# ColumbiaDVMM/ColumbiaImageSearch

Hardware: AMD Instinct MI355X
Metric: queries/sec @ recall@10 on 10M LOPQ index (higher is better)
Workload: dtype f64

## Files before the change

columbiaimagesearch_amd/csrc/lopq_scan3.hip:

```cpp
#include "scan_common.h"
#include <cmath>
#include <cstdio>
#include <cstdlib>

typedef unsigned short u16x2_t __attribute__((ext_vector_type(2)));

static __device__ __forceinline__ uint32_t pk_add_u16(uint32_t a, uint32_t b) {
    return __builtin_bit_cast(uint32_t, (u16x2_t)(__builtin_bit_cast(u16x2_t, a) + __builtin_bit_cast(u16x2_t, b)));
}
static __device__ __forceinline__ uint32_t pk_subsat_u16(uint32_t a, uint32_t b) {
    return __builtin_bit_cast(uint32_t, __builtin_elementwise_sub_sat(__builtin_bit_cast(u16x2_t, a), __builtin_bit_cast(u16x2_t, b)));
}

static __device__ __forceinline__ uint32_t pk_min_u16(uint32_t a, uint32_t b) {
    return __builtin_bit_cast(uint32_t, __builtin_elementwise_min(__builtin_bit_cast(u16x2_t, a), __builtin_bit_cast(u16x2_t, b)));
}

static const int S3G = 4;

#ifdef CIS_S3_COUNTERS
__device__ unsigned long long g_s3_ctr[16];
#define S3_CLK() ((long long)__builtin_amdgcn_s_memtime())
#define S3_CTR(i, v) do { if (threadIdx.x == 0) atomicAdd(&g_s3_ctr[i], (unsigned long long)(v)); } while (0)
extern "C" int cis_debug_counters3(unsigned long long* out, int reset) {
// ... 561 lines not shown
            for (int g = 0; g < G; ++g) {
                const uint32_t sg = (g & 1) ? (d[u][g >> 1] >> 16) : (d[u][g >> 1] & 0xffffu);
                const uint32_t t1 = (g & 1) ? ((g >> 1) ? s23 >> 16 : s01 >> 16) : ((g >> 1) ? s23 & 0xffffu : s01 & 0xffffu);
                pm[u][g] = __ballot(sg < t1) & anym[u];
                if (any_dup) {
                    bool same = true;
#pragma unroll
                    for (int i = 0; i < (M + 3) / 4; ++i) same = same && (cur[u].w[i] == dup[g].w[i]);
                    pm[u][g] &= ~(__ballot(same) & (has_dup[g] ? ~0ull : 0ull));
                }
            }
        }
#pragma unroll
        for (int g = 0; g < G; ++g) {
            if (g >= ng) break;
            uint32_t* rk = rk_all + (g * NW + w) * R;
            int ntot = 0;
#pragma unroll
            for (int u = 0; u < U; ++u) ntot += __popcll(pm[u][g]);
            if (ntot == 0) continue;
            auto entry = [&](int u) -> uint32_t {
                const uint32_t sg = (g & 1) ? (d[u][g >> 1] >> 16) : (d[u][g >> 1] & 0xffffu);
                return (sg << 16) | (uint32_t)(base + u * 64 + lane);
            };
            if (cnt[g] + ntot <= R) {
                int c = cnt[g];
#pragma unroll
                for (int u = 0; u < U; ++u) {
                    const unsigned long long m = pm[u][g];
                    if (m == 0ull) continue;
                    const int idx = __builtin_amdgcn_mbcnt_hi((unsigned)(m >> 32), __builtin_amdgcn_mbcnt_lo((unsigned)m, c));
                    if ((m >> lane) & 1ull) rk[idx] = entry(u);
                    c += __popcll(m);
                }
                cnt[g] = c;
                continue;
            }
            int u0 = 0;
            while (true) {
                bool full = false;
#pragma unroll
                for (int u = 0; u < U; ++u) {
                    const unsigned long long m = pm[u][g];
                    if (u < u0 || full || m == 0ull) continue;
                    const int n = __popcll(m);
                    if (cnt[g] + n > R) {
                        full = true;
                        u0 = u;
                        continue;
                    }
                    const int idx = cnt[g] + __builtin_amdgcn_mbcnt_hi((unsigned)(m >> 32), __builtin_amdgcn_mbcnt_lo((unsigned)m, 0));
                    if ((m >> lane) & 1ull) rk[idx] = entry(u);
                    cnt[g] += n;
                    u0 = u + 1;
                }
                if (!full) break;
                const QScale qsg = load_scale(&sh[g]);
                int c2 = wave_compact3<M, NR, NW>(rk, cnt[g], L, Lw, R - 64, qsg, &sh[g], w);
                if (c2 < 0) {
                    uint32_t dp = 0xffffffffu;
                    const WorkItem itg = items[item_idx[g]];
                    c2 = wave_compact3_exact<M, NR, NW>(rk, cnt[g], L, Lw, qsg, &sh[g], w, codes, start, K,
                                                        T + (int64_t)itg.tab0 * nf * K, T + (int64_t)itg.tab1 * nf * K, dp);
                    dp = (uint32_t)__builtin_amdgcn_readfirstlane((int)dp);
                    if (dp != 0xffffffffu) {
                        dup[g] = load_code<M>(codes, start + (int64_t)dp);
                        has_dup[g] = true;
                        any_dup = true;
                    }
                }
                cnt[g] = c2;
                const uint32_t thg = lds_ld(&sh[g].thr);
                if (lane == 0) st16(&thr1[g], thg + 1u);
                const unsigned long long dup_on = has_dup[g] ? ~0ull : 0ull;
#pragma unroll
                for (int u = 0; u < U; ++u) {
                    const uint32_t sg = (g & 1) ? (d[u][g >> 1] >> 16) : (d[u][g >> 1] & 0xffffu);
                    bool same = true;
#pragma unroll
                    for (int i = 0; i < (M + 3) / 4; ++i) same = same && (cur[u].w[i] == dup[g].w[i]);
                    pm[u][g] &= __ballot(sg <= thg) & ~(__ballot(same) & dup_on);
                }
            }
        }
    }
    S3_CTR(4, S3_CLK() - c0);
#pragma unroll
    for (int g = 0; g < G; ++g) {
        if (g >= ng) break;
        uint32_t* rk = rk_all + (g * NW + w) * R;
        if (cnt[g] > 0) cnt[g] = wave_compact3<M, NR, NW>(rk, cnt[g], L, Lw, NR * 64, load_scale(&sh[g]), &sh[g], w);
    }
    S3_CTR(5, S3_CLK() - c0);
    if constexpr (NW > 1) __syncthreads();
    S3_CTR(6, S3_CLK() - c0);
#pragma unroll
    for (int g = 0; g < G; ++g) {
        if (g >= ng) break;
        uint32_t* rk = rk_all + (g * NW + w) * R;
        const QScale qsg = load_scale(&sh[g]);
        if constexpr (NW > 1) cnt[g] = wave_filter3<NR, NW>(rk, cnt[g], qsg, &sh[g]);
        if (lane == 0) sh[g].wcnt[w] = cnt[g];
        if (tid == 0) {
            const uint64_t b = block_bound<NW>(&sh[g]);
            if (b < sh[g].ext) atomicMin(&qbound[items[item_idx[g]].q], (unsigned long long)b);
        }
    }
    if constexpr (NW > 1) __syncthreads();
#pragma unroll
    for (int g = 0; g < G; ++g) {
        if (g >= ng) break;
        const uint32_t* rk = rk_all + (g * NW + w) * R;
        int off = 0, total = 0;
#pragma unroll
        for (int i = 0; i < NW; ++i) {
            const int c = (NW > 1) ? sh[g].wcnt[i] : cnt[g];
            off += (i < w) ? c : 0;
            total += c;
        }
        uint64_t* out = item_surv + (int64_t)item_idx[g] * S + off;
        for (int e = lane; e < cnt[g]; e += 64) {
            const uint32_t x = rk[e];
            out[e] = ((uint64_t)(x >> 16) << 32) | (x & 0xffffu);
        }
        if (tid == 0) item_n[item_idx[g]] = total;
    }
    S3_CTR(7, S3_CLK() - c0);
    S3_CTR(0, 1);
}

template <int M, int NR, int U, int NW, int WPE>
__global__ __launch_bounds__(NW * 64) __attribute__((amdgpu_waves_per_eu(WPE, WPE))) void k_adc_scan3(
    const WorkItem* __restrict__ items, const TabDesc* __restrict__ tabs, const int* __restrict__ slots,
    const int* __restrict__ n_slots_ptr, const double* __restrict__ T, const float* __restrict__ T32,
    const uint8_t* __restrict__ codes, int K, int L, int S, int* __restrict__ queue_ctr ,
    uint64_t* __restrict__ item_surv, int* __restrict__ item_n, float* __restrict__ item_slack,
    unsigned long long* __restrict__ qbound , int two_pass, int single_queue ) {
    extern __shared__ __attribute__((aligned(16))) char smem[];
    constexpr int G = S3G;
    constexpr int R = NR * 64 - 8;
    int* s_next = reinterpret_cast<int*>(smem + (size_t)K * M * G * 2 + (size_t)G * NW * R * 4 + G * sizeof(Scan3Shared) + 32);
    const int* qs = n_slots_ptr + 8;
    const int home = blockIdx.x & 7;
    const long long k0 = S3_CLK();
    (void)k0;
    for (int a = 0; a < 8; ++a) {
        const int x = (home + a) & 7;
        const int qstart = qs[x];
        const int count = single_queue ? (x == 0 ? qs[1] - qstart : 0) : qs[x + 1] - qstart;
        if (count <= 0) continue;
        while (true) {
            const long long q0 = S3_CLK();
            (void)q0;
            int j;
            if constexpr (NW > 1) {
                __syncthreads();
                if (threadIdx.x == 0) *s_next = atomicAdd(&queue_ctr[x], 1);
                __syncthreads();
                j = __builtin_amdgcn_readfirstlane(*s_next);
            } else {
                int t = 0;
                if (threadIdx.x == 0) t = atomicAdd(&queue_ctr[x], 1);
                j = __builtin_amdgcn_readfirstlane(t);
            }
            S3_CTR(8, S3_CLK() - q0);
            if (j >= count) break;
            const int slot = qstart + j;
            int idx[G];
            int ng = 0;
            bool same = true;
#pragma unroll
            for (int g = 0; g < G; ++g) {
                idx[g] = slots[slot * G + g];
                if (idx[g] >= 0) {
                    ng = g + 1;
                    same = same && items[idx[g]].start == items[idx[0]].start && items[idx[g]].len == items[idx[0]].len;
                } else {
                    idx[g] = idx[0];
                }
            }
            if (!same) {
                for (int g2 = 0; g2 < ng; ++g2) {
                    int oi[G];
#pragma unroll
                    for (int g = 0; g < G; ++g) {
                        oi[g] = idx[0];
#pragma unroll
                        for (int gg = 1; gg < G; ++gg)
                            if (gg == g2) oi[g] = idx[gg];
                    }
                    if (g2 > 0) __syncthreads();
                    scan3_group<M, NR, U, NW>(items, tabs, oi, 1, T, T32, codes, K, L, S, item_surv, item_n, item_slack, qbound, smem, two_pass != 0);
                }
                continue;
            }
            scan3_group<M, NR, U, NW>(items, tabs, idx, ng, T, T32, codes, K, L, S, item_surv, item_n, item_slack, qbound, smem, two_pass != 0);
        }
    }
    S3_CTR(9, S3_CLK() - k0);
    S3_CTR(10, 1);
}

struct Slot4 {
    int item[S3G], tab0[S3G], tab1[S3G], q[S3G];
    float qinv[S3G];
    int start_lo, start_hi, len, ng;
    int ist_lo[S3G], ist_hi[S3G], ilen[S3G];
};
struct Scan4Shared {
    double inv_up, ub;
    uint64_t ext;
    uint32_t tau;
    int verify;
    int cnt;
    int q;
};

template <int M, int UU, int OCT = (M >= 8 ? 8 : 4)>
__device__ __forceinline__ void adc16_rows(const CodeWords<M> (&cur)[UU], const char* __restrict__ tab, const RotConsts<M>& rc,
                                           u32x2_t (&d)[UU]) {
    constexpr int NU = M / OCT;
    u32x2_t fbuf[2][OCT];
    uint32_t D[2][(M + 3) / 4];
    rot_words<M>(cur[0], rc, D[0]);
    adc16_issue<M, OCT>(D[0], 0, tab, rc, fbuf[0]);
#pragma unroll
    for (int q = 0; q < UU * NU; ++q) {
        const int u = q / NU, o = q % NU;
        if (q + 1 < UU * NU) {
            const int u1 = (q + 1) / NU, o1 = (q + 1) % NU;
            if (o1 == 0) rot_words<M>(cur[u1], rc, D[u1 & 1]);
            adc16_issue<M, OCT>(D[u1 & 1], o1, tab, rc, fbuf[(q + 1) & 1]);
        }
        __builtin_amdgcn_sched_barrier(0);
        const u32x2_t part = adc16_sum<OCT>(fbuf[q & 1]);
        if (o == 0) {
            d[u] = part;
        } else {
            d[u][0] = pk_add_u16(d[u][0], part[0]);
            d[u][1] = pk_add_u16(d[u][1], part[1]);
        }
        __builtin_amdgcn_sched_barrier(0);
    }
}

static __device__ __forceinline__ void lds_barrier() {
    asm volatile("s_waitcnt lgkmcnt(0)\n\ts_barrier" ::: "memory");
}

#ifndef CIS_S4_U
#define CIS_S4_U 2
#endif
#ifndef CIS_S4_UL
#define CIS_S4_UL 2
#endif
#ifndef CIS_S4_OCT
#define CIS_S4_OCT 4
#endif
#ifndef CIS_S4_WPE
#define CIS_S4_WPE 6
#endif
static const int S4_OCT = CIS_S4_OCT;
#ifndef CIS_S4_DEFER
#define CIS_S4_DEFER 1
#endif
#ifndef CIS_S4_NW_LONG
#define CIS_S4_NW_LONG 4
#endif
#ifndef CIS_S4_NW_SHORT
#define CIS_S4_NW_SHORT 4
#endif
#ifndef CIS_S4_WPE8
#define CIS_S4_WPE8 6
#endif
#ifndef CIS_S4_GLISTS
#define CIS_S4_GLISTS 0
#endif
#ifndef CIS_S4_WPE_LONG
#define CIS_S4_WPE_LONG 6
#endif
#ifndef CIS_S4_PF
#define CIS_S4_PF 2
#endif
#ifndef CIS_S4_LCAP
#define CIS_S4_LCAP 504
#endif
#ifndef CIS_S4_NS
#define CIS_S4_NS 16
#endif
#ifndef CIS_S4_Z
#define CIS_S4_Z 4.0f
#endif
static const int S4_DS = 8;
static const int S4_LCAP = CIS_S4_LCAP;
static const int S4_NS = CIS_S4_NS;

static const int S4_LCAP_LONG = 1016;

static size_t scan4_lds(int M, int K, int lcap, int nw) {
    const bool glists = lcap > 504 && CIS_S4_DEFER != 0 && CIS_S4_GLISTS != 0;
    const size_t lists = glists ? (size_t)nw * ((32 / nw) * 128) * 2 : (size_t)S3G * lcap * 4, samp = glists ? 0 : (size_t)S3G * S4_NS * 64 * 2;
    return (size_t)K * M * S3G * 2 + (lists > samp ? lists : samp) + S3G * sizeof(Scan4Shared) + 32 + (size_t)S3G * nw * 4 + (S4_DS + 1) * sizeof(Slot4);
}

template <int M, int U, int NW, int WPE, int LCAPT>
__global__ __launch_bounds__(NW * 64) __attribute__((amdgpu_waves_per_eu(WPE, WPE))) void k_adc_scan4(
    const WorkItem* __restrict__ items, const TabDesc* __restrict__ tabs, const int* __restrict__ slots,
    const int* __restrict__ n_slots_ptr, const float* __restrict__ T32 , const double* __restrict__ T,
    const uint8_t* __restrict__ codes, int K, int L, int S,
    int* __restrict__ dbg , int* __restrict__ fhdr ,
    int* __restrict__ fslots, uint64_t* __restrict__ item_surv, int* __restrict__ item_n, float* __restrict__ item_slack,
    unsigned long long* __restrict__ qbound, float zq , int frac_den ,
    int nsx , int dyn ,
    float sat ) {
    extern __shared__ __attribute__((aligned(16))) char smem[];
    constexpr int G = S3G;
    static_assert(NW >= G && NW % G == 0 && NW <= 8, "waves 0 .. G-1 serve one query each in the threshold and verification phases");
    static_assert(M == 4 || M == 8 || M == 16, "float4s of the half tables are dealt to the threads in rounds of 256");
    constexpr int nf = M / 2;
    constexpr uint32_t CAP = 65535u / M;
    constexpr int LCAP = LCAPT, NS = S4_NS, NRV = (LCAP + 63) / 64;
    constexpr bool GLISTS = (LCAPT > 504) && (CIS_S4_DEFER != 0) && (CIS_S4_GLISTS != 0);
    constexpr size_t LIST_B_FULL = (size_t)G * LCAP * 4 > (size_t)G * NS * 64 * 2 ? (size_t)G * LCAP * 4 : (size_t)G * NS * 64 * 2;
    constexpr size_t LIST_B = GLISTS ? (size_t)NW * (((LCAPT > 504 ? 32 : 16) / NW) * 128) * 2 : LIST_B_FULL;
    char* tab = smem;
    uint32_t* lists = reinterpret_cast<uint32_t*>(smem + (size_t)K * M * G * 2);
    uint16_t* samp = reinterpret_cast<uint16_t*>(lists);
    Scan4Shared* sh = reinterpret_cast<Scan4Shared*>(reinterpret_cast<char*>(lists) + LIST_B);
    uint16_t* thr1 = reinterpret_cast<uint16_t*>(sh + G);
    int* s_flag = reinterpret_cast<int*>(thr1 + 4);
    int* s_cnt = s_flag + 1;
    int* wcnt = reinterpret_cast<int*>(reinterpret_cast<char*>(thr1) + 32);
    Slot4* sd = reinterpret_cast<Slot4*>(reinterpret_cast<char*>(thr1) + 32 + G * NW * 4);
#ifdef CIS_S4_SHARED_LISTS
    constexpr bool WLISTS = LCAPT > 504;
#else
    constexpr bool WLISTS = true;
#endif
    constexpr int WCAP = LCAPT / NW;
    constexpr int PCAP_LDS = (int)(LIST_B / (NW * 2));
    constexpr int NRP = (LCAPT > 504 ? 32 : 16) / NW;
    constexpr int PCAP = NRP * 128 < PCAP_LDS ? NRP * 128 : PCAP_LDS;
    static_assert(PCAP % 2 == 0 && (PCAP_LDS * 2) % 4 == 0, "position lists are read back as 32-bit pairs");
    const int tid = threadIdx.x, lane = tid & 63;
    const int w = __builtin_amdgcn_readfirstlane(tid >> 6);
    const int total = n_slots_ptr[0];
    const int xcd = blockIdx.x & 7, lb = blockIdx.x >> 3;
    const int LW = gridDim.x >> 3;
    auto slot_of = [&](int k) -> int {
        const int li = lb + k * LW;
        const int j = (((li >> 5) * 8 + xcd) << 5) | (li & 31);
        return j < total ? j : -1;
    };
    const RotConsts<M> rc = make_rot<M>(lane);
    const int nvec = (nf * K) >> 2;
    const long long k0 = S3_CLK();
    (void)k0;
    for (int kb = 0;; kb += S4_DS) {
        int dyn_j = -1;
        if (LCAPT > 504 && dyn) {
            __syncthreads();
            if (tid == 0) {
                int jn = -1;
                if (dyn == 1) {
                    jn = atomicAdd(&dbg[6], 1);
                    jn = jn < total ? jn : -1;
                } else {
                    int* qx = dbg - 9;
                    for (int a2 = 0; a2 < 8 && jn < 0; ++a2) {
                        const int x = (xcd + a2) & 7;
                        const int li = atomicAdd(&qx[x], 1);
                        const int jj = (((li >> 5) * 8 + x) << 5) | (li & 31);
                        if (jj < total) jn = jj;
                    }
                }
                *s_flag = jn;
            }
            __syncthreads();
            dyn_j = *s_flag;
            if (dyn_j < 0) break;
        } else {
            if (slot_of(kb) < 0) break;
        }
        __syncthreads();
        if (tid < S4_DS) {
            Slot4 d;
            const int j = (LCAPT > 504 && dyn) ? (tid == 0 ? dyn_j : -1) : slot_of(kb + tid);
            d.ng = 0; d.len = 0; d.start_lo = d.start_hi = 0;
#pragma unroll
            for (int g = 0; g < G; ++g) { d.item[g] = 0; d.tab0[g] = 0; d.tab1[g] = 0; d.q[g] = 0; d.qinv[g] = 0.f; d.ist_lo[g] = d.ist_hi[g] = d.ilen[g] = 0; }
            if (j >= 0) {
                int idx[G];
                int ng = 0;
                bool same = true;
#pragma unroll
                for (int g = 0; g < G; ++g) idx[g] = slots[j * G + g];
                const int64_t st0 = items[idx[0]].start;
                const int len0 = items[idx[0]].len;
#pragma unroll
                for (int g = 0; g < G; ++g) {
                    if (idx[g] >= 0) ng = g + 1;
                    else idx[g] = idx[0];
                    const WorkItem* it = &items[idx[g]];
                    same = same && it->start == st0 && it->len == len0;
                    const int t0 = it->tab0, t1 = it->tab1;
                    d.item[g] = idx[g]; d.tab0[g] = t0; d.tab1[g] = t1; d.q[g] = it->q;
                    d.ist_lo[g] = (int)(uint32_t)it->start; d.ist_hi[g] = (int)(it->start >> 32); d.ilen[g] = it->len;
                    float mxT = fmaxf(__int_as_float(tabs[t0].pad), __int_as_float(tabs[t1].pad));
                    mxT = fmaxf(mxT, 1e-30f);
                    float qi = ((float)CAP / mxT) * (1.0f - 9.5367431640625e-7f);
                    qi = (mxT < 3.0e38f) ? qi : 0.0f;
                    qi = (qi < 3.0e38f) ? qi : 3.0e38f;
                    d.qinv[g] = qi;
                }
                d.start_lo = (int)(uint32_t)st0; d.start_hi = (int)(st0 >> 32); d.len = len0;
                d.ng = same ? ng : -ng;
            }
            sd[tid] = d;
        }
        __syncthreads();
        for (int kk = 0; kk < S4_DS; ++kk) {
            const Slot4* d = &sd[kk];
            const int ngs0 = __builtin_amdgcn_readfirstlane(d->ng);
            if (ngs0 == 0) break;
            int remaining = ngs0 < 0 ? ((1 << (-ngs0)) - 1) : 0;
            do {
            if (ngs0 < 0) {
                Slot4* ds = &sd[S4_DS];
                if (tid == 0) {
                    const Slot4* src = &sd[kk];
                    int g0 = 0;
                    while (!((remaining >> g0) & 1)) ++g0;
                    int n = 0, rest = remaining;
                    for (int h = g0; h < G; ++h) {
                        if (((remaining >> h) & 1) && src->ist_lo[h] == src->ist_lo[g0] && src->ist_hi[h] == src->ist_hi[g0] && src->ilen[h] == src->ilen[g0]) {
                            ds->item[n] = src->item[h]; ds->tab0[n] = src->tab0[h]; ds->tab1[n] = src->tab1[h]; ds->q[n] = src->q[h];
                            ds->qinv[n] = src->qinv[h];
                            ++n;
                            rest &= ~(1 << h);
                        }
                    }
                    for (int h = n; h < G; ++h) {
                        ds->item[h] = ds->item[0]; ds->tab0[h] = ds->tab0[0]; ds->tab1[h] = ds->tab1[0]; ds->q[h] = ds->q[0]; ds->qinv[h] = ds->qinv[0];
                    }
                    ds->start_lo = src->ist_lo[g0]; ds->start_hi = src->ist_hi[g0]; ds->len = src->ilen[g0];
                    ds->ng = n;
                    ds->ist_lo[0] = rest;
                }
                lds_barrier();
                d = ds;
                remaining = __builtin_amdgcn_readfirstlane(ds->ist_lo[0]);
            }
            const int ngs = __builtin_amdgcn_readfirstlane(d->ng);
            const long long c0 = S3_CLK();
            (void)c0;
            const int ng = ngs;
            bool fail = false;
            if (!fail) {
                float qinv[G];
#pragma unroll
                for (int g = 0; g < G; ++g)
                    qinv[g] = __builtin_bit_cast(float, __builtin_amdgcn_readfirstlane(__builtin_bit_cast(int, d->qinv[g])));
                const int len = __builtin_amdgcn_readfirstlane(d->len);
                const int64_t start = ((int64_t)__builtin_amdgcn_readfirstlane(d->start_hi) << 32) | (uint32_t)__builtin_amdgcn_readfirstlane(d->start_lo);
                if (sat > 0.0f) {
                    if (w < G) {
                        const int g = w;
                        if (g < ng) {
                            const int t0 = __builtin_amdgcn_readfirstlane(d->tab0[g]), t1 = __builtin_amdgcn_readfirstlane(d->tab1[g]);
                            const int64_t Ta = (int64_t)t0 * nf * K, Tb = (int64_t)t1 * nf * K;
                            const int c = len >= 64 ? (int)(((int64_t)lane * len) >> 6) : lane;
                            uint32_t key = 0x7f7fffffu;
                            if (c < len) {
                                const CodeWords<M> cw = load_code<M>(codes, start + c);
                                float ds = 0.f;
#pragma unroll
                                for (int j = 0; j < M / 2; ++j) ds += tab_f1(T32, T, Ta + j * K + ((cw.w[j >> 2] >> (8 * (j & 3))) & 255u));
#pragma unroll
                                for (int j = 0; j < M / 2; ++j) ds += tab_f1(T32, T, Tb + j * K + ((cw.w[(M / 2 + j) >> 2] >> (8 * ((M / 2 + j) & 3))) & 255u));
                                key = __float_as_uint(fmaxf(ds, 0.f));
                            }
                            int rk = 4 + (int)((64 * (int64_t)L + len - 1) / len);
                            rk = rk > 48 ? 48 : rk;
                            uint32_t mn = key;
                            for (int r = 0; r < rk; ++r) {
                                uint32_t mx = 0u;
                                mn = key;
                                wave_minmax_step<1>(mn, mx); wave_minmax_step<2>(mn, mx); wave_minmax_step<4>(mn, mx);
                                wave_minmax_step<8>(mn, mx); wave_minmax_step<16>(mn, mx); wave_minmax_step<32>(mn, mx);
                                if (r + 1 < rk) {
                                    const uint64_t hit = __ballot(key == mn);
                                    if (lane == (int)__builtin_ctzll(hit)) key = 0x7f7fffffu;
                                }
                            }
                            const float d4 = __uint_as_float(mn);
                            const float qs = (sat * (float)CAP) / fmaxf(d4, 1e-30f);
                            const float q0 = d->qinv[g];
                            if (lane == 0 && q0 > 0.0f && qs > q0 && qs < 3.0e38f && d4 < 1.0e38f) const_cast<Slot4*>(d)->qinv[g] = qs;
                        }
                    }
                    lds_barrier();
#pragma unroll
                    for (int g = 0; g < G; ++g)
                        qinv[g] = __builtin_bit_cast(float, __builtin_amdgcn_readfirstlane(__builtin_bit_cast(int, d->qinv[g])));
                }
                int tid_st = tid;
                asm volatile("" : "+v"(tid_st));
                for (int vt = tid_st; vt < nvec; vt += NW * 64) {
                    const int j = vt & (nf - 1), kq = vt / nf, k0 = 4 * kq;
                    const int vidx = j * (K >> 2) + kq;
                    float4 pv[G][2];
#pragma unroll
                    for (int g = 0; g < G; ++g) {
                        const int t0 = __builtin_amdgcn_readfirstlane(d->tab0[g]), t1 = __builtin_amdgcn_readfirstlane(d->tab1[g]);
                        pv[g][0] = tab_f4(T32, T, t0, nf * K, vidx);
                        pv[g][1] = tab_f4(T32, T, t1, nf * K, vidx);
                    }
                    uint32_t* tw = reinterpret_cast<uint32_t*>(tab);
#pragma unroll
                    for (int s2 = 0; s2 < 2; ++s2) {
#pragma unroll
                        for (int c = 0; c < 4; ++c) {
                            uint32_t qv[G];
#pragma unroll
                            for (int g = 0; g < G; ++g) {
                                const float4 q = pv[g][s2];
                                const float x = c == 0 ? q.x : (c == 1 ? q.y : (c == 2 ? q.z : q.w));
                                qv[g] = (g < ng) ? (uint32_t)(x * qinv[g]) : CAP;
                                qv[g] = qv[g] > CAP ? CAP : qv[g];
                            }
                            u32x2_t pk;
                            pk[0] = qv[0] | (qv[1] << 16);
                            pk[1] = qv[2] | (qv[3] << 16);
                            *reinterpret_cast<u32x2_t*>(tw + (((k0 + c) * M + s2 * nf + j) << 1)) = pk;
                        }
                    }
                }
                if (tid >= 64 && tid < 64 + G) {
                    const int g = tid - 64;
                    float qi = qinv[0];
#pragma unroll
                    for (int gg = 1; gg < G; ++gg) qi = (g == gg) ? qinv[gg] : qi;
                    const double inv_up = (double)qi * (1.0 + 2.384185791015625e-7);
                    const double ub = qi > 0.0f ? (1.0 + 4.76837158203125e-7) / (double)qi : __longlong_as_double(0x7ff0000000000000LL);
                    const int item = d->item[g];
                    const int q = d->q[g];
                    sh[g].inv_up = inv_up;
                    sh[g].ub = ub;
                    sh[g].q = q;
                    sh[g].ext = (g < ng) ? __hip_atomic_load(&qbound[q], __ATOMIC_RELAXED, __HIP_MEMORY_SCOPE_AGENT) : 0x7ff0000000000000ull;
                    sh[g].cnt = 0;
                    s_cnt[g] = 0;
                    if (g < ng) {
                        item_slack[2 * (int64_t)item + 0] = __double2float_ru(ub * ((double)M + 0.1));
                        item_slack[2 * (int64_t)item + 1] = __double2float_ru(ub);
                    }
                }
                if (tid == 0) *s_flag = 0;
                __amdgpu_buffer_rsrc_t rs;
                {
                    const uint64_t cbase = (uint64_t)(uintptr_t)(codes + start * M);
                    const uint32_t blo = (uint32_t)__builtin_amdgcn_readfirstlane((int)(uint32_t)cbase);
                    const uint32_t bhi = (uint32_t)__builtin_amdgcn_readfirstlane((int)(uint32_t)(cbase >> 32));
                    rs = __builtin_amdgcn_make_buffer_rsrc((void*)(uintptr_t)(((uint64_t)bhi << 32) | blo), 0, len * M, 0x00020000);
                }
                const int nrows = (len + 63) >> 6;
                constexpr bool MULTI = LCAPT > 504;
                if constexpr (!MULTI) {
                    const int ns = nrows < NS ? nrows : NS;
                    constexpr int SPW = NS / NW;
                    static_assert(NS % (2 * NW) == 0, "sample rows come in pairs per wave");
                    CodeWords<M> sc[SPW];
                    int srow[SPW];
#pragma unroll
                    for (int i = 0; i < SPW; ++i) {
                        const int t = SPW * w + i;
                        srow[i] = t < ns ? (int)(((int64_t)t * nrows) / ns) : nrows;
                        sc[i] = load_code_buf<M>(rs, srow[i] * 64 + lane);
                    }
                    S3_CTR(11, S3_CLK() - c0);
                    lds_barrier();
                    S3_CTR(2, S3_CLK() - c0);
                    {
                        u32x2_t dd[SPW];
#if defined(CIS_S4_PROBE) && CIS_S4_PROBE >= 3
                        for (int u = 0; u < SPW; ++u) { dd[u][0] = 0xffffffffu; dd[u][1] = 0xffffffffu; }
#else
                        adc16_rows<M, SPW, S4_OCT>(sc, tab, rc, dd);
#endif
#pragma unroll
                        for (int u = 0; u < SPW; ++u) {
                            const int t = SPW * w + u;
                            const bool ok = (t < ns) && (srow[u] * 64 + lane < len);
#pragma unroll
                            for (int g = 0; g < G; ++g) {
                                const uint32_t sg = (g & 1) ? (dd[u][g >> 1] >> 16) : (dd[u][g >> 1] & 0xffffu);
#if defined(CIS_S4_PROBE) && CIS_S4_PROBE >= 3
                                samp[g * (NS * 64) + t * 64 + lane] = (uint16_t)0xffffu;
#else
                                samp[g * (NS * 64) + t * 64 + lane] = (uint16_t)(ok ? sg : 0xffffu);
#endif
                            }
                        }
                    }
                    lds_barrier();
                    S3_CTR(3, S3_CLK() - c0);
                    if (w < G) {
                        const int g = w;
                        uint32_t sv[NS];
                        int nsam = 0;
#pragma unroll
                        for (int r = 0; r < NS; ++r) {
                            sv[r] = samp[g * (NS * 64) + r * 64 + lane];
                            nsam += __popcll(__ballot(sv[r] != 0xffffu));
                        }
                        const bool exact = ns == nrows;
                        int ksv = L;
                        if (!exact) {
                            const float need = (float)L * (float)nsam / (float)len;
                            const float hz = 0.5f * zq;
                            const float rt = hz + sqrtf(hz * hz + need);
                            ksv = (int)(rt * rt) + 1;
                        }
                        uint32_t tau = 65534u;
                        bool have_bound = false;
                        if (g < ng && nsam >= ksv) {
                            uint32_t lo = 0u, hi = 65534u;
                            while (lo < hi) {
                                const uint32_t p = lo + ((hi - lo) >> 1);
                                int c = 0;
#pragma unroll
                                for (int r = 0; r < NS; ++r) c += __popcll(__ballot(sv[r] <= p));
                                if (c >= ksv) hi = p;
                                else lo = p + 1;
                            }
                            tau = lo;
                            have_bound = tau < (sat > 0.f ? CAP - (uint32_t)M - 2u : 65534u);
                        }
                        if (lane == 0) {
                            uint32_t keep = 65534u;
                            if (have_bound) {
                                keep = tau + (uint32_t)M + 1u;
                                keep = keep < 65534u ? keep : 65534u;
                            }
                            const uint32_t t_ext = (g < ng) ? bound_to_thr(sh[g].ext, sh[g].inv_up) : 0u;
                            const uint32_t t = keep < t_ext ? keep : t_ext;
                            thr1[g] = (uint16_t)((g < ng) ? t + 1u : 0u);
#if defined(CIS_S4_PROBE) && CIS_S4_PROBE == 1
                            thr1[g] = 0;
#endif
                            sh[g].tau = tau;
                            sh[g].verify = (have_bound && keep < t_ext && !exact) ? 1 : 0;
#if defined(CIS_S4_PROBE)
                            sh[g].verify = 0;
#endif
                        }
                    }
                } else {
                    int ns = nrows / frac_den;
                    ns = ns < NS ? NS : ns;
                    ns = ns > nsx ? nsx : ns;
                    ns = ns < nrows ? ns : nrows;
                    constexpr int SPW = 4;
                    const int rounds = (ns + NW * SPW - 1) / (NW * SPW);
                    CodeWords<M> sc[SPW];
                    int srow[SPW];
#pragma unroll
                    for (int i = 0; i < SPW; ++i) {
                        const int t = SPW * w + i;
                        srow[i] = t < ns ? (int)(((int64_t)t * nrows) / ns) : nrows;
                        sc[i] = load_code_buf<M>(rs, srow[i] * 64 + lane);
                    }
                    S3_CTR(11, S3_CLK() - c0);
                    lds_barrier();
                    S3_CTR(2, S3_CLK() - c0);
                    {
                        uint32_t bm0 = 0xffffffffu, bm1 = 0xffffffffu;
#pragma unroll 1
                        for (int r = 0; r < rounds; ++r) {
                            CodeWords<M> nsc[SPW];
                            int nrow[SPW];
                            if constexpr (MULTI) {
                                if (r + 1 < rounds) {
#pragma unroll
                                    for (int i = 0; i < SPW; ++i) {
                                        const int t = ((r + 1) * NW + w) * SPW + i;
                                        nrow[i] = t < ns ? (int)(((int64_t)t * nrows) / ns) : nrows;
                                        nsc[i] = load_code_buf<M>(rs, nrow[i] * 64 + lane);
                                    }
                                }
                            }
                            u32x2_t dd[SPW];
#if defined(CIS_S4_PROBE) && CIS_S4_PROBE >= 3
                            for (int u = 0; u < SPW; ++u) { dd[u][0] = 0xffffffffu; dd[u][1] = 0xffffffffu; }
#else
                            adc16_rows<M, SPW, S4_OCT>(sc, tab, rc, dd);
#endif
#pragma unroll
                            for (int u = 0; u < SPW; ++u) {
                                const bool ok = srow[u] < nrows && (srow[u] * 64 + lane < len);
                                bm0 = pk_min_u16(bm0, ok ? dd[u][0] : 0xffffffffu);
                                bm1 = pk_min_u16(bm1, ok ? dd[u][1] : 0xffffffffu);
                            }
                            if constexpr (MULTI) {
                                if (r + 1 < rounds) {
#pragma unroll
                                    for (int i = 0; i < SPW; ++i) { sc[i] = nsc[i]; srow[i] = nrow[i]; }
                                }
                            }
                        }
                        u32x2_t bm;
                        bm[0] = bm0; bm[1] = bm1;
                        reinterpret_cast<u32x2_t*>(samp)[w * 64 + lane] = bm;
                    }
                    lds_barrier();
                    S3_CTR(3, S3_CLK() - c0);
                    if (w < G) {
                        const int g = w;
                        uint32_t sv[NW];
#pragma unroll
                        for (int r = 0; r < NW; ++r) {
                            const u32x2_t x = reinterpret_cast<const volatile u32x2_t*>(samp)[r * 64 + lane];
                            const uint32_t xw = (g >> 1) ? x[1] : x[0];
                            sv[r] = (g & 1) ? (xw >> 16) : (xw & 0xffffu);
                        }
                        const bool all = ns == nrows;
                        const int nsam = all ? len : ns * 64;
                        int ksv = L;
                        if (!all) {
                            const float need = (float)L * (float)nsam / (float)len;
                            const float hz = 0.5f * zq;
                            const float rt = hz + sqrtf(hz * hz + need);
                            ksv = (int)(rt * rt) + 1;
                        }
                        uint32_t tau = 65534u;
                        bool have_bound = false;
                        if (g < ng && nsam >= ksv) {
                            uint32_t lo = 0u, hi = 65534u;
                            while (lo < hi) {
                                const uint32_t p = lo + ((hi - lo) >> 1);
                                int c = 0;
#pragma unroll
                                for (int r = 0; r < NW; ++r) c += __popcll(__ballot(sv[r] <= p));
                                if (c >= ksv) hi = p;
                                else lo = p + 1;
                            }
                            tau = lo;
                            have_bound = tau < (sat > 0.f ? CAP - (uint32_t)M - 2u : 65534u);
                        }
                        if (lane == 0) {
                            uint32_t keep = 65534u;
                            if (have_bound) {
                                keep = tau + (uint32_t)M + 1u;
                                keep = keep < 65534u ? keep : 65534u;
                            }
                            const uint32_t t_ext = (g < ng) ? bound_to_thr(sh[g].ext, sh[g].inv_up) : 0u;
                            const uint32_t t = keep < t_ext ? keep : t_ext;
                            thr1[g] = (uint16_t)((g < ng) ? t + 1u : 0u);
#if defined(CIS_S4_PROBE) && CIS_S4_PROBE == 1
                            thr1[g] = 0;
#endif
                            sh[g].tau = tau;
                            sh[g].verify = (have_bound && keep < t_ext && !all) ? 1 : 0;
#if defined(CIS_S4_PROBE)
                            sh[g].verify = 0;
#endif
                        }
                    }
                }
                lds_barrier();
                S3_CTR(4, S3_CLK() - c0);
                {
                    const u32x2_t tpk = *reinterpret_cast<const volatile u32x2_t*>(thr1);
                    const uint32_t s01 = (uint32_t)__builtin_amdgcn_readfirstlane((int)tpk[0]);
                    const uint32_t s23 = (uint32_t)__builtin_amdgcn_readfirstlane((int)tpk[1]);
#if defined(CIS_S4_PROBE) && CIS_S4_PROBE >= 2
                    const int nit = 0;
#else
                    const int nit = (len + 64 * U - 1) / (64 * U);
#endif
                    constexpr int PF = CIS_S4_PF;
                    CodeWords<M> ring[PF][U];
#pragma unroll
                    for (int k = 0; k < PF; ++k) {
#pragma unroll
                        for (int u = 0; u < U; ++u) ring[k][u] = load_code_buf<M>(rs, (w + k * NW) * 64 * U + u * 64 + lane);
                        __builtin_amdgcn_sched_barrier(0);
                    }
                    int wcur[G];
#pragma unroll
                    for (int g = 0; g < G; ++g) wcur[g] = 0;
#if CIS_S4_DEFER
                    uint16_t* plist = reinterpret_cast<uint16_t*>(lists) + (size_t)w * PCAP_LDS;
                    int pcur = 0;
#endif
                    for (int iter0 = w; iter0 < nit; iter0 += NW * PF) {
#pragma unroll
                      for (int k = 0; k < PF; ++k) {
                        const int iter = iter0 + k * NW;
                        const int base = iter * 64 * U;
                        u32x2_t dd[U];
                        adc16_rows<M, U, S4_OCT>(ring[k], tab, rc, dd);
#pragma unroll
                        for (int u = 0; u < U; ++u) ring[k][u] = load_code_buf<M>(rs, (iter + PF * NW) * 64 * U + u * 64 + lane);
#pragma unroll
                        for (int u = 0; u < U; ++u) {
                            const uint32_t xx = pk_subsat_u16(tpk[0], dd[u][0]) | pk_subsat_u16(tpk[1], dd[u][1]);
                            unsigned long long am = __ballot(xx != 0u);
                            const int n = len - base - u * 64;
                            if (n < 64) am &= n <= 0 ? 0ull : ((1ull << n) - 1ull);
                            if (am == 0ull) continue;
#if CIS_S4_DEFER
                            if constexpr (WLISTS) {
                                const int idx = __builtin_amdgcn_mbcnt_hi((unsigned)(am >> 32), __builtin_amdgcn_mbcnt_lo((unsigned)am, pcur));
                                if (((am >> lane) & 1ull) && idx < PCAP) plist[idx] = (uint16_t)(base + u * 64 + lane);
                                pcur += __popcll(am);
                                continue;
                            }
#endif
                            if constexpr (WLISTS) {
#ifdef CIS_S4_SCALAR_APPEND
                                while (am != 0ull) {
                                    const int l = __builtin_ctzll(am);
                                    am &= am - 1ull;
                                    const uint32_t d0 = (uint32_t)__builtin_amdgcn_readlane((int)dd[u][0], l);
                                    const uint32_t d1 = (uint32_t)__builtin_amdgcn_readlane((int)dd[u][1], l);
                                    const uint32_t pos = (uint32_t)(base + u * 64 + l);
#pragma unroll
                                    for (int g = 0; g < G; ++g) {
                                        const uint32_t dw = (g >> 1) ? d1 : d0;
                                        const uint32_t sg = (g & 1) ? (dw >> 16) : (dw & 0xffffu);
                                        const uint32_t t1 = (g & 1) ? ((g >> 1) ? s23 >> 16 : s01 >> 16) : ((g >> 1) ? s23 & 0xffffu : s01 & 0xffffu);
                                        if (sg < t1) {
                                            if (wcur[g] < WCAP) lists[(g * NW + w) * WCAP + wcur[g]] = (sg << 16) | pos;
                                            wcur[g] += 1;
                                        }
                                    }
                                }
#else
#pragma unroll
                                for (int g = 0; g < G; ++g) {
                                    const uint32_t sg = (g & 1) ? (dd[u][g >> 1] >> 16) : (dd[u][g >> 1] & 0xffffu);
                                    const uint32_t t1 = (g & 1) ? ((g >> 1) ? s23 >> 16 : s01 >> 16) : ((g >> 1) ? s23 & 0xffffu : s01 & 0xffffu);
                                    const unsigned long long mg = __ballot(sg < t1) & am;
                                    if (mg == 0ull) continue;
                                    const int idx = __builtin_amdgcn_mbcnt_hi((unsigned)(mg >> 32), __builtin_amdgcn_mbcnt_lo((unsigned)mg, wcur[g]));
                                    if (((mg >> lane) & 1ull) && idx < WCAP) lists[(g * NW + w) * WCAP + idx] = (sg << 16) | (uint32_t)(base + u * 64 + lane);
                                    wcur[g] += __popcll(mg);
                                }
#endif
                                continue;
                            }
                            unsigned long long m[G];
                            int mine = 0;
#pragma unroll
                            for (int g = 0; g < G; ++g) {
                                const uint32_t sg = (g & 1) ? (dd[u][g >> 1] >> 16) : (dd[u][g >> 1] & 0xffffu);
                                const uint32_t t1 = (g & 1) ? ((g >> 1) ? s23 >> 16 : s01 >> 16) : ((g >> 1) ? s23 & 0xffffu : s01 & 0xffffu);
                                m[g] = __ballot(sg < t1) & am;
                                mine = (lane == g) ? __popcll(m[g]) : mine;
                            }
                            int got = 0;
                            if (lane < G) got = atomicAdd(&s_cnt[lane], mine);
#pragma unroll
                            for (int g = 0; g < G; ++g) {
                                if (m[g] == 0ull) continue;
                                const int b0 = __builtin_amdgcn_readlane(got, g);
                                const uint32_t sg = (g & 1) ? (dd[u][g >> 1] >> 16) : (dd[u][g >> 1] & 0xffffu);
                                const int idx = __builtin_amdgcn_mbcnt_hi((unsigned)(m[g] >> 32), __builtin_amdgcn_mbcnt_lo((unsigned)m[g], b0));
                                if (((m[g] >> lane) & 1ull) && idx < LCAP) lists[g * LCAP + idx] = (sg << 16) | (uint32_t)(base + u * 64 + lane);
                            }
                        }
                      }
                    }
                    S3_CTR(13, S3_CLK() - c0);
#if CIS_S4_DEFER
                    if constexpr (WLISTS) {
                        const bool pover = pcur > PCAP;
                        const int pn = pover ? 0 : pcur;
                        uint32_t pp[NRP];
#pragma unroll
                        for (int r = 0; r < NRP; ++r)
                            pp[r] = (2 * (r * 64) < pn) ? reinterpret_cast<const volatile uint32_t*>(plist)[r * 64 + lane] : 0u;
                        lds_barrier();
                        uint32_t* grow[G];
#pragma unroll
                        for (int g = 0; g < G; ++g)
                            grow[g] = reinterpret_cast<uint32_t*>(item_surv + (int64_t)__builtin_amdgcn_readfirstlane(d->item[g]) * S);
                        if (pn > 0) {
                            auto pos_of = [&](int it) -> uint32_t {
                                uint32_t v = pp[0];
#pragma unroll
                                for (int r = 1; r < NRP; ++r) v = ((it >> 1) == r) ? pp[r] : v;
                                return (it & 1) ? (v >> 16) : (v & 0xffffu);
                            };
                            auto on_of = [&](int it) -> bool { return 2 * (((it >> 1) * 64) + lane) + (it & 1) < pn; };
                            const int nit2 = 2 * ((pn + 127) >> 7);
                            CodeWords<M> nxc[1];
                            uint32_t npos = pos_of(0);
                            nxc[0] = load_code_buf<M>(rs, on_of(0) ? (int)npos : len);
#pragma unroll 1
                            for (int it = 0; it < nit2; ++it) {
                                CodeWords<M> cc[1];
                                cc[0] = nxc[0];
                                const uint32_t pos = npos;
                                const bool on = on_of(it);
                                if (it + 1 < nit2) {
                                    npos = pos_of(it + 1);
                                    nxc[0] = load_code_buf<M>(rs, on_of(it + 1) ? (int)npos : len);
                                }
                                u32x2_t d1[1];
                                adc16_rows<M, 1, S4_OCT>(cc, tab, rc, d1);
                                const unsigned long long am2 = __ballot(on);
#pragma unroll
                                for (int g = 0; g < G; ++g) {
                                    const uint32_t sg = (g & 1) ? (d1[0][g >> 1] >> 16) : (d1[0][g >> 1] & 0xffffu);
                                    const uint32_t t1 = (g & 1) ? ((g >> 1) ? s23 >> 16 : s01 >> 16) : ((g >> 1) ? s23 & 0xffffu : s01 & 0xffffu);
                                    const unsigned long long mg = __ballot(sg < t1) & am2;
                                    if (mg == 0ull) continue;
                                    const int idx = __builtin_amdgcn_mbcnt_hi((unsigned)(mg >> 32), __builtin_amdgcn_mbcnt_lo((unsigned)mg, wcur[g]));
                                    if (((mg >> lane) & 1ull) && idx < WCAP) {
                                        if constexpr (GLISTS) grow[g][w * WCAP + idx] = (sg << 16) | pos;
                                        else lists[(g * NW + w) * WCAP + idx] = (sg << 16) | pos;
                                    }
                                    wcur[g] += __popcll(mg);
                                }
                            }
                        }
                        if (pover) wcur[0] = WCAP + 1;
                    }
#endif
                    if constexpr (WLISTS) {
                        if (lane < G) {
                            int c = wcur[0];
#pragma unroll
                            for (int g = 1; g < G; ++g) c = (lane == g) ? wcur[g] : c;
                            wcnt[lane * NW + w] = c;
                        }
                    }
                }
                S3_CTR(12, S3_CLK() - c0);
                if constexpr (GLISTS) __syncthreads();
                else lds_barrier();
                S3_CTR(5, S3_CLK() - c0);
                bool bad = false;
                if (w < ng) {
                    const int g = w;
                    int tot = 0;
                    int wtot[NW];
                    int lane_v = lane;
                    asm volatile("" : "+v"(lane_v));
                    if constexpr (WLISTS) {
#pragma unroll
                        for (int r = 0; r < NW; ++r) {
                            wtot[r] = wcnt[g * NW + r];
                            bad = bad || wtot[r] > WCAP;
                            tot += wtot[r];
                        }
                    } else {
                        tot = s_cnt[g];
                        bad = tot > LCAP;
                    }
                    if (bad && lane_v == 0) atomicAdd(&dbg[2], 1);
                    if (!bad) {
                        uint32_t ent[NRV];
                        bool val[NRV];
#pragma unroll
                        for (int r = 0; r < NRV; ++r) {
                            if constexpr (WLISTS) {
                                constexpr int RW = NRV / NW;
                                const int e = (r % RW) * 64 + lane_v;
                                val[r] = e < wtot[r / RW];
                                if constexpr (GLISTS) {
                                    const uint32_t* gr = reinterpret_cast<const uint32_t*>(item_surv + (int64_t)__builtin_amdgcn_readfirstlane(d->item[g]) * S);
                                    ent[r] = val[r] ? __hip_atomic_load(gr + (r / RW) * WCAP + e, __ATOMIC_RELAXED, __HIP_MEMORY_SCOPE_AGENT) : 0xffffffffu;
                                } else {
                                    ent[r] = val[r] ? lists[(g * NW + r / RW) * WCAP + e] : 0xffffffffu;
                                }
                            } else {
                                val[r] = r * 64 + lane_v < tot;
                                ent[r] = val[r] ? lists[g * LCAP + r * 64 + lane_v] : 0xffffffffu;
                            }
                        }
                        const uint32_t tau = sh[g].tau;
                        if (sh[g].verify) {
                            int nle = 0;
#pragma unroll
                            for (int r = 0; r < NRV; ++r) nle += __popcll(__ballot(val[r] && (ent[r] >> 16) <= tau));
                            bad = nle < L;
                            if (bad && lane_v == 0) atomicAdd(&dbg[3], 1);
                        }
                        if (!bad) {
                            uint32_t cut = 65535u;
                            if (tot >= L) {
                                uint32_t mn = 0xffffffffu, mx = 0u;
#pragma unroll
                                for (int r = 0; r < NRV; ++r) {
                                    const uint32_t s = ent[r] >> 16;
                                    mn = (val[r] && s < mn) ? s : mn;
                                    mx = (val[r] && s > mx) ? s : mx;
                                }
                                wave_minmax_all(mn, mx);
                                uint32_t lo = mn, hi = mx;
                                while (lo < hi) {
                                    const uint32_t p = lo + ((hi - lo) >> 1);
                                    int c = 0;
#pragma unroll
                                    for (int r = 0; r < NRV; ++r) c += __popcll(__ballot(val[r] && (ent[r] >> 16) <= p));
                                    if (c >= L) {
                                        hi = p;
                                        if (c <= L + 16) break;
                                    } else {
                                        lo = p + 1;
                                    }
                                }
                                cut = hi + (uint32_t)M + 1u;
                                if (sat > 0.f && cut >= CAP) {
                                    bad = true;
                                    if (lane_v == 0) atomicAdd(&dbg[4], 1);
                                }
                                const uint64_t b = val_to_bound(hi, M, sh[g].ub);
                                if (lane_v == 0 && !bad && b < sh[g].ext) atomicMin(&qbound[sh[g].q], (unsigned long long)b);
                            } else if (sat > 0.f) {
                                bool sat = false;
#pragma unroll
                                for (int r = 0; r < NRV; ++r) sat = sat || (__ballot(val[r] && (ent[r] >> 16) + (uint32_t)M + 1u >= CAP) != 0ull);
                                if (sat) {
                                    bad = true;
                                    if (lane_v == 0) atomicAdd(&dbg[4], 1);
                                }
                            }
                            const int item = __builtin_amdgcn_readfirstlane(d->item[g]);
                            uint64_t* out = item_surv + (int64_t)item * S;
                            if constexpr (LCAP > 504) {
                                int nk = 0;
#pragma unroll
                                for (int r = 0; r < NRV; ++r) nk += __popcll(__ballot(val[r] && (ent[r] >> 16) <= cut));
                                if (nk > S) {
                                    bad = true;
                                    if (lane_v == 0) atomicAdd(&dbg[4], 1);
                                }
                            }
                            if (!bad) {
                                int kept = 0;
#pragma unroll
                                for (int r = 0; r < NRV; ++r) {
                                    const bool kp = val[r] && (ent[r] >> 16) <= cut;
                                    const unsigned long long mk = __ballot(kp);
                                    const int idx = kept + __builtin_amdgcn_mbcnt_hi((unsigned)(mk >> 32), __builtin_amdgcn_mbcnt_lo((unsigned)mk, 0));
                                    if (kp) out[idx] = ((uint64_t)(ent[r] >> 16) << 32) | (ent[r] & 0xffffu);
                                    kept += __popcll(mk);
                                }
                                if (lane_v == 0) item_n[item] = kept;
                            }
                        }
                    }
                    if (bad && lane_v == 0) *s_flag = 1;
                }
                lds_barrier();
                S3_CTR(6, S3_CLK() - c0);
                fail = *s_flag != 0;
            }
            S3_CTR(0, 1);
            if (tid == 0) {
                atomicAdd(&dbg[0], 1);
                if (ngs0 < 0) atomicAdd(&dbg[5], 1);
                if (fail) {
                    atomicAdd(&dbg[1], 1);
                    const int f = atomicAdd(&fhdr[17], 1);
#pragma unroll
                    for (int g = 0; g < G; ++g) fslots[f * G + g] = g < ng ? d->item[g] : -1;
                }
            }
            } while (remaining != 0);
        }
    }
    S3_CTR(9, S3_CLK() - k0);
    S3_CTR(10, 1);
}

static const int S5G = 8;
typedef unsigned int u32x4v __attribute__((ext_vector_type(4)));

template <int M, int OCT>
__device__ __forceinline__ void adc16x8_issue(const uint32_t (&D)[(M + 3) / 4], int o, const char* __restrict__ tab, const RotConsts<M>& rc,
                                              u32x4v (&f)[OCT]) {
    constexpr int SH = ((M == 4) ? 2 : (M == 8 ? 3 : 4)) + 4;
#pragma unroll
    for (int i = 0; i < OCT; ++i) {
        const int t = o * OCT + i;
        const uint32_t k = __builtin_amdgcn_ubfe(D[t >> 2], rc.sh[t & 3], 8);
        f[i] = *reinterpret_cast<const u32x4v*>(tab + ((k << SH) | (rc.cj[t] << 2)));
    }
}

template <int OCT>
__device__ __forceinline__ u32x4v adc16x8_sum(const u32x4v (&f)[OCT]) {
    u32x4v a = f[0];
#pragma unroll
    for (int i = 1; i < OCT; ++i) {
        a[0] = pk_add_u16(a[0], f[i][0]);
        a[1] = pk_add_u16(a[1], f[i][1]);
        a[2] = pk_add_u16(a[2], f[i][2]);
        a[3] = pk_add_u16(a[3], f[i][3]);
    }
    return a;
}

template <int M, int UU, int OCT>
__device__ __forceinline__ void adc16x8_rows(const CodeWords<M> (&cur)[UU], const char* __restrict__ tab, const RotConsts<M>& rc, u32x4v (&d)[UU]) {
    constexpr int NU = M / OCT;
    u32x4v fbuf[2][OCT];
    uint32_t D[2][(M + 3) / 4];
    rot_words<M>(cur[0], rc, D[0]);
    adc16x8_issue<M, OCT>(D[0], 0, tab, rc, fbuf[0]);
#pragma unroll
    for (int q = 0; q < UU * NU; ++q) {
        const int u = q / NU, o = q % NU;
        if (q + 1 < UU * NU) {
            const int u1 = (q + 1) / NU, o1 = (q + 1) % NU;
            if (o1 == 0) rot_words<M>(cur[u1], rc, D[u1 & 1]);
            adc16x8_issue<M, OCT>(D[u1 & 1], o1, tab, rc, fbuf[(q + 1) & 1]);
        }
        __builtin_amdgcn_sched_barrier(0);
        const u32x4v part = adc16x8_sum<OCT>(fbuf[q & 1]);
        if (o == 0) {
            d[u] = part;
        } else {
#pragma unroll
            for (int x = 0; x < 4; ++x) d[u][x] = pk_add_u16(d[u][x], part[x]);
        }
        __builtin_amdgcn_sched_barrier(0);
    }
}

struct Slot5 {
    int item[S5G], tab0[S5G], tab1[S5G], q[S5G];
    float qinv[S5G];
    uint32_t thr1[S5G], ok1[S5G];
    float ubf[S5G];
    int start_lo, start_hi, len, ng, same;
};

static __device__ __forceinline__ uint32_t s5_sum_of(const u32x4v& d, int g) {
    const uint32_t w = d[g >> 1];
    return (g & 1) ? (w >> 16) : (w & 0xffffu);
}

static const int S5_PCAP = 1024;

static size_t scan5_lds(int M, int K) { return (size_t)K * M * S5G * 2 + (size_t)4 * S5_PCAP * 2 + sizeof(Slot5) + 64; }

template <int M, bool SAMPLE, int WPE>
__global__ __launch_bounds__(256) __attribute__((amdgpu_waves_per_eu(WPE, WPE))) void k_adc_scan5(
    const WorkItem* __restrict__ items, const TabDesc* __restrict__ tabs, const int* __restrict__ slots, const int* __restrict__ n_slots_ptr,
    const float* __restrict__ T32 , const double* __restrict__ T, const uint8_t* __restrict__ codes, int K, int S,
    const float* __restrict__ tau, uint32_t* __restrict__ bmin, int B, int* __restrict__ nsamp, int ss,
    uint64_t* __restrict__ item_surv, int* __restrict__ item_n, float* __restrict__ item_slack, int* __restrict__ cnt_ok, int* __restrict__ ovf) {
    extern __shared__ __attribute__((aligned(16))) char smem[];
    constexpr int G = S5G, NW = 4, nf = M / 2, U = 2, PF = 2, OCT = 4;
    constexpr uint32_t CAP = 65535u / M;
    char* tab = smem;
    uint16_t* plist_all = reinterpret_cast<uint16_t*>(smem + (size_t)K * M * G * 2);
    Slot5* sd = reinterpret_cast<Slot5*>(reinterpret_cast<char*>(plist_all) + (size_t)NW * S5_PCAP * 2);
    const int tid = threadIdx.x, lane = tid & 63;
    const int w = __builtin_amdgcn_readfirstlane(tid >> 6);
    const int total = n_slots_ptr[0];
    const int xcd = blockIdx.x & 7, lb = blockIdx.x >> 3, LW = gridDim.x >> 3;
    const RotConsts<M> rc = make_rot<M>(lane);
    const int nvec = (nf * K) >> 2;
    for (int kk = 0;; ++kk) {
        const int li = lb + kk * LW;
        const int j = (((li >> 5) * 8 + xcd) << 5) | (li & 31);
        if ((li >> 5) * 256 >= total + 256) break;
        if (j >= total) continue;
        __syncthreads();
        if (tid < G) {
            const int g = tid;
            int idx = slots[j * G + g];
            const int idx0 = slots[j * G];
            const bool on = idx >= 0;
            idx = on ? idx : idx0;
            const WorkItem it = items[idx];
            const WorkItem it0 = items[idx0];
            float mxT = fmaxf(__int_as_float(tabs[it.tab0].pad), __int_as_float(tabs[it.tab1].pad));
            mxT = fmaxf(mxT, 1e-30f);
            float qi = ((float)CAP / mxT) * (1.0f - 9.5367431640625e-7f);
            qi = (mxT < 3.0e38f) ? qi : 0.0f;
            qi = (qi < 3.0e38f) ? qi : 3.0e38f;
            sd->item[g] = idx; sd->tab0[g] = it.tab0; sd->tab1[g] = it.tab1; sd->q[g] = on ? it.q : -1;
            sd->qinv[g] = qi;
            const double inv_up = (double)qi * (1.0 + 2.384185791015625e-7);
            const double ub = qi > 0.0f ? (1.0 + 4.76837158203125e-7) / (double)qi : __longlong_as_double(0x7ff0000000000000LL);
            sd->ubf[g] = __double2float_ru(ub);
            uint32_t t1 = 0u, o1 = 0u;
            if (on && !SAMPLE) {
                const float tq = tau[it.q];
                if (!(tq < 3.0e38f)) { t1 = 65535u; o1 = 65535u; }
                else {
                    const double x = (double)tq * inv_up;
                    t1 = x >= 65533.0 ? 65535u : (uint32_t)x + 2u;
                    const double y = (double)tq / ((double)sd->ubf[g]) - (double)M - 1.0;
                    o1 = y <= 0.0 ? 0u : (y >= 65533.0 ? 65535u : (uint32_t)y + 1u);
                }
            }
            sd->thr1[g] = t1; sd->ok1[g] = o1;
            if (on && !SAMPLE) {
                item_slack[2 * (int64_t)idx + 0] = __double2float_ru(ub * ((double)M + 0.1));
                item_slack[2 * (int64_t)idx + 1] = __double2float_ru(ub);
            }
            const bool same = it.start == it0.start && it.len == it0.len;
            const unsigned long long sm = __ballot(same || !on);
            if (g == 0) {
                sd->start_lo = (int)(uint32_t)it0.start; sd->start_hi = (int)(it0.start >> 32); sd->len = it0.len;
                sd->same = ((sm & 0xffull) == 0xffull) ? 1 : 0;
            }
            const unsigned long long om = __ballot(on);
            if (g == 0) sd->ng = 64 - __builtin_clzll((om & 0xffull) | 0ull) ;
        }
        __syncthreads();
        const int ng = __builtin_amdgcn_readfirstlane(sd->ng);
        const int len = __builtin_amdgcn_readfirstlane(sd->len);
        const int64_t start = ((int64_t)__builtin_amdgcn_readfirstlane(sd->start_hi) << 32) | (uint32_t)__builtin_amdgcn_readfirstlane(sd->start_lo);
        if (!__builtin_amdgcn_readfirstlane(sd->same)) {
            if (!SAMPLE && tid < ng && sd->q[tid] >= 0) ovf[sd->q[tid]] = 1;
            continue;
        }
        {
            float qinv[G];
// ... 374 lines not shown
```

Measured before the change: 22.84 million.

## Restructure survivor verification loop with two-deep code prefetch and shifted position registers

Rewrites the position-list verification loop so each register holds two positions, and the code words for the next pair are loaded two iterations ahead, replacing the per-iteration select chain over NRP registers with a register shift. The first code loads are issued before the LDS barrier so the memory latency overlaps the barrier. Several volatile LDS reads become non-volatile lds_ld calls, the sample-row division uses 32-bit unsigned arithmetic, and empty asm constraints pin scalar and vector values to particular register classes. The change costs extra registers for the second in-flight code buffer, and the unconditional reads from the position list rely on the new static_assert bound.

```diff
diff --git a/columbiaimagesearch_amd/csrc/lopq_scan3.hip b/columbiaimagesearch_amd/csrc/lopq_scan3.hip
--- a/columbiaimagesearch_amd/csrc/lopq_scan3.hip
+++ b/columbiaimagesearch_amd/csrc/lopq_scan3.hip
@@ -887,6 +887,8 @@
     const size_t lists = glists ? (size_t)nw * ((32 / nw) * 128) * 2 : (size_t)S3G * lcap * 4, samp = glists ? 0 : (size_t)S3G * S4_NS * 64 * 2;
     return (size_t)K * M * S3G * 2 + (lists > samp ? lists : samp) + S3G * sizeof(Scan4Shared) + 32 + (size_t)S3G * nw * 4 + (S4_DS + 1) * sizeof(Slot4);
 }
+
+static __device__ __forceinline__ int sample_row(int t, int nrows, int ns) { return (int)(((uint32_t)t * (uint32_t)nrows) / (uint32_t)ns); }
 
 template <int M, int U, int NW, int WPE, int LCAPT>
 __global__ __launch_bounds__(NW * 64) __attribute__((amdgpu_waves_per_eu(WPE, WPE))) void k_adc_scan4(
@@ -970,7 +972,9 @@
         __syncthreads();
         if (tid < S4_DS) {
             Slot4 d;
-            const int j = (LCAPT > 504 && dyn) ? (tid == 0 ? dyn_j : -1) : slot_of(kb + tid);
+            int dyn_s = dyn;
+            asm volatile("" : "+s"(dyn_s));
+            const int j = (LCAPT > 504 && dyn_s) ? (tid == 0 ? dyn_j : -1) : slot_of(kb + tid);
             d.ng = 0; d.len = 0; d.start_lo = d.start_hi = 0;
 #pragma unroll
             for (int g = 0; g < G; ++g) { d.item[g] = 0; d.tab0[g] = 0; d.tab1[g] = 0; d.q[g] = 0; d.qinv[g] = 0.f; d.ist_lo[g] = d.ist_hi[g] = d.ilen[g] = 0; }
@@ -1001,7 +1005,9 @@
                 d.start_lo = (int)(uint32_t)st0; d.start_hi = (int)(st0 >> 32); d.len = len0;
                 d.ng = same ? ng : -ng;
             }
-            sd[tid] = d;
+            int tid_d = tid;
+            asm volatile("" : "+v"(tid_d));
+            sd[tid_d] = d;
         }
         __syncthreads();
         for (int kk = 0; kk < S4_DS; ++kk) {
@@ -1160,7 +1166,7 @@
 #pragma unroll
                     for (int i = 0; i < SPW; ++i) {
                         const int t = SPW * w + i;
-                        srow[i] = t < ns ? (int)(((int64_t)t * nrows) / ns) : nrows;
+                        srow[i] = t < ns ? sample_row(t, nrows, ns) : nrows;
                         sc[i] = load_code_buf<M>(rs, srow[i] * 64 + lane);
                     }
                     S3_CTR(11, S3_CLK() - c0);
@@ -1203,7 +1209,9 @@
                         int ksv = L;
                         if (!exact) {
                             const float need = (float)L * (float)nsam / (float)len;
-                            const float hz = 0.5f * zq;
+                            float zq_s = zq;
+                            asm volatile("" : "+s"(zq_s));
+                            const float hz = 0.5f * zq_s;
                             const float rt = hz + sqrtf(hz * hz + need);
                             ksv = (int)(rt * rt) + 1;
                         }
@@ -1253,7 +1261,7 @@
 #pragma unroll
                     for (int i = 0; i < SPW; ++i) {
                         const int t = SPW * w + i;
-                        srow[i] = t < ns ? (int)(((int64_t)t * nrows) / ns) : nrows;
+                        srow[i] = t < ns ? sample_row(t, nrows, ns) : nrows;
                         sc[i] = load_code_buf<M>(rs, srow[i] * 64 + lane);
                     }
                     S3_CTR(11, S3_CLK() - c0);
@@ -1270,7 +1278,7 @@
 #pragma unroll
                                     for (int i = 0; i < SPW; ++i) {
                                         const int t = ((r + 1) * NW + w) * SPW + i;
-                                        nrow[i] = t < ns ? (int)(((int64_t)t * nrows) / ns) : nrows;
+                                        nrow[i] = t < ns ? sample_row(t, nrows, ns) : nrows;
                                         nsc[i] = load_code_buf<M>(rs, nrow[i] * 64 + lane);
                                     }
                                 }
@@ -1305,8 +1313,7 @@
                         uint32_t sv[NW];
 #pragma unroll
                         for (int r = 0; r < NW; ++r) {
-                            const u32x2_t x = reinterpret_cast<const volatile u32x2_t*>(samp)[r * 64 + lane];
-                            const uint32_t xw = (g >> 1) ? x[1] : x[0];
+                            const uint32_t xw = lds_ld(reinterpret_cast<const uint32_t*>(samp) + 2 * (r * 64 + lane) + (g >> 1));
                             sv[r] = (g & 1) ? (xw >> 16) : (xw & 0xffffu);
                         }
                         const bool all = ns == nrows;
@@ -1356,7 +1363,9 @@
                 lds_barrier();
                 S3_CTR(4, S3_CLK() - c0);
                 {
-                    const u32x2_t tpk = *reinterpret_cast<const volatile u32x2_t*>(thr1);
+                    const uint64_t tp64 = lds_ld(reinterpret_cast<const uint64_t*>(thr1));
+                    u32x2_t tpk;
+                    tpk[0] = (uint32_t)tp64; tpk[1] = (uint32_t)(tp64 >> 32);
                     const uint32_t s01 = (uint32_t)__builtin_amdgcn_readfirstlane((int)tpk[0]);
                     const uint32_t s23 = (uint32_t)__builtin_amdgcn_readfirstlane((int)tpk[1]);
 #if defined(CIS_S4_PROBE) && CIS_S4_PROBE >= 2
@@ -1463,40 +1472,37 @@
                     if constexpr (WLISTS) {
                         const bool pover = pcur > PCAP;
                         const int pn = pover ? 0 : pcur;
+                        static_assert(NRP * 128 <= PCAP_LDS, "the NRP registers are read from the wave's own position list");
                         uint32_t pp[NRP];
 #pragma unroll
-                        for (int r = 0; r < NRP; ++r)
-                            pp[r] = (2 * (r * 64) < pn) ? reinterpret_cast<const volatile uint32_t*>(plist)[r * 64 + lane] : 0u;
+                        for (int r = 0; r < NRP; ++r) pp[r] = lds_ld(reinterpret_cast<const uint32_t*>(plist) + r * 64 + lane);
+                        auto on_of = [&](int it) -> bool { return 2 * (((it >> 1) * 64) + lane) + (it & 1) < pn; };
+                        CodeWords<M> cw[2];
+                        cw[0] = load_code_buf<M>(rs, on_of(0) ? (int)(pp[0] & 0xffffu) : len);
+                        cw[1] = load_code_buf<M>(rs, on_of(1) ? (int)(pp[0] >> 16) : len);
                         lds_barrier();
                         uint32_t* grow[G];
 #pragma unroll
                         for (int g = 0; g < G; ++g)
                             grow[g] = reinterpret_cast<uint32_t*>(item_surv + (int64_t)__builtin_amdgcn_readfirstlane(d->item[g]) * S);
                         if (pn > 0) {
-                            auto pos_of = [&](int it) -> uint32_t {
-                                uint32_t v = pp[0];
-#pragma unroll
-                                for (int r = 1; r < NRP; ++r) v = ((it >> 1) == r) ? pp[r] : v;
-                                return (it & 1) ? (v >> 16) : (v & 0xffffu);
-                            };
-                            auto on_of = [&](int it) -> bool { return 2 * (((it >> 1) * 64) + lane) + (it & 1) < pn; };
-                            const int nit2 = 2 * ((pn + 127) >> 7);
-                            CodeWords<M> nxc[1];
-                            uint32_t npos = pos_of(0);
-                            nxc[0] = load_code_buf<M>(rs, on_of(0) ? (int)npos : len);
+                            const int nreg = (pn + 127) >> 7;
 #pragma unroll 1
-                            for (int it = 0; it < nit2; ++it) {
+                            for (int r = 0; r < nreg; ++r) {
+                              const uint32_t cur = pp[0];
+#pragma unroll
+                              for (int k = 0; k + 1 < NRP; ++k) pp[k] = pp[k + 1];
+                              pp[NRP - 1] = 0u;
+#pragma unroll
+                              for (int h = 0; h < 2; ++h) {
+                                const int it = 2 * r + h;
+                                const uint32_t pos = h ? (cur >> 16) : (cur & 0xffffu);
                                 CodeWords<M> cc[1];
-                                cc[0] = nxc[0];
-                                const uint32_t pos = npos;
-                                const bool on = on_of(it);
-                                if (it + 1 < nit2) {
-                                    npos = pos_of(it + 1);
-                                    nxc[0] = load_code_buf<M>(rs, on_of(it + 1) ? (int)npos : len);
-                                }
+                                cc[0] = cw[h];
                                 u32x2_t d1[1];
                                 adc16_rows<M, 1, S4_OCT>(cc, tab, rc, d1);
-                                const unsigned long long am2 = __ballot(on);
+                                cw[h] = load_code_buf<M>(rs, on_of(it + 2) ? (int)(h ? (pp[0] >> 16) : (pp[0] & 0xffffu)) : len);
+                                const unsigned long long am2 = __ballot(on_of(it));
 #pragma unroll
                                 for (int g = 0; g < G; ++g) {
                                     const uint32_t sg = (g & 1) ? (d1[0][g >> 1] >> 16) : (d1[0][g >> 1] & 0xffffu);
@@ -1510,6 +1516,7 @@
                                     }
                                     wcur[g] += __popcll(mg);
                                 }
+                              }
                             }
                         }
                         if (pover) wcur[0] = WCAP + 1;
```

New measurement: 23.77 million, median of 6. 4.1% higher.
